# osqp/OSQP.jl

Measured on AMD Instinct MI355X. Metric: ADMM iterations/sec, higher is better.
Workload: dtype f64; 1 GPU; rand-1e6; n=1000000, m=1000000, nnz_A=1000000000, nnz_P_full=1000749500, nnz_P_triu=500874750, backend=pcg, check_termination=25, adaptive_rho_interval=50, instances=1

## Files before the change

include/osqp_amd.h:

```cpp
#ifndef OSQP_AMD_H
#define OSQP_AMD_H

#include <stddef.h>

#ifdef __cplusplus
extern "C" {
#endif

typedef long long c_int;
typedef double    c_float;

#define OSQP_INFTY 1e30

enum osqp_linsys_solver_type {
  QDLDL_SOLVER       = 0,
  MKL_PARDISO_SOLVER = 1,
  AMD_PCG_SOLVER     = 2,
  AMD_DIRECT_SOLVER  = 3
};

#define OSQP_DUAL_INFEASIBLE_INACCURATE    (4)
#define OSQP_PRIMAL_INFEASIBLE_INACCURATE  (3)
#define OSQP_SOLVED_INACCURATE             (2)
#define OSQP_SOLVED                        (1)
// ... 190 lines not shown

c_int osqp_warm_start_x(OSQPWorkspace *work, const c_float *x);
c_int osqp_warm_start_y(OSQPWorkspace *work, const c_float *y);
c_int osqp_warm_start(OSQPWorkspace *work, const c_float *x, const c_float *y);


enum osqp_amd_problem_kind {
  OSQP_AMD_GEN_RANDOM_QP = 0,
  OSQP_AMD_GEN_LASSO     = 1,
  OSQP_AMD_GEN_MPC       = 2
};

c_int osqp_amd_setup_generated(OSQPWorkspace **workp, c_int kind, c_int n, c_int per_row,
                               unsigned long long seed, const OSQPSettings *settings);

#define OSQP_AMD_STATS_COUNT 26
c_int osqp_amd_get_stats(const OSQPWorkspace *work, c_float *out, c_int count);

c_float osqp_amd_time_kernel(OSQPWorkspace *work, c_int which, c_int reps);

typedef struct osqp_amd_comm osqp_amd_comm;
typedef int (*osqp_amd_allgather_fn)(void *ctx, double *host_buf, long long count);
c_int osqp_amd_comm_create_host(osqp_amd_comm **out, c_int rank, c_int world, osqp_amd_allgather_fn fn, void *ctx);
c_int osqp_amd_comm_unique_id(void *out128, const char *librccl_path);
c_int osqp_amd_comm_create_rccl(osqp_amd_comm **out, c_int rank, c_int world, const void *unique_id,
                                const char *librccl_path);
c_int osqp_amd_comm_destroy(osqp_amd_comm *comm);
c_int osqp_amd_comm_all_gather(osqp_amd_comm *comm, c_float *dev_buf, c_int count);
c_int osqp_amd_comm_info(const osqp_amd_comm *comm, c_int *rank, c_int *world, c_int *transport_ranks);
c_int osqp_amd_setup_sharded(OSQPWorkspace **workp, const OSQPData *data, const OSQPSettings *settings,
                             osqp_amd_comm *comm);
// ... 130 lines not shown
```

osqp.jl_amd/csrc/abi.hip:

```cpp
#include "engine.hpp"
#include "symbolic.hpp"

#include <cstring>
#include <thread>
#include <atomic>
#include <cmath>

using namespace oq;

namespace {

struct Impl {
  Engine eng;
  OSQPData data;
  OSQPSettings settings;
  OSQPSolution solution;
  OSQPInfo info;
};

Engine *E(OSQPWorkspace *w) { return &((Impl *)w->impl)->eng; }

struct DeviceGuard {
  int prev = -1;
  explicit DeviceGuard(int want) {
// ... 664 lines not shown
  v[11] = e.lin->trisolve_bytes();
  v[12] = e.A.panel.active ? (e.A.panel.wide ? 3.0 : 2.0) : 0.0;
  v[13] = e.comm ? (c_float)e.comm->world : 1.0;
  v[14] = e.comm ? e.comm->exchanges : 0.0;
  v[15] = e.comm ? e.comm->bytes : 0.0;
  v[16] = (c_float)e.n;
  v[17] = (c_float)e.m;
  v[18] = e.compact ? 1.0 : 0.0;
  v[19] = e.lin->supernode_levels();
  v[20] = (c_float)g_device_peak;
  v[21] = (c_float)e.tree_restarts;
  v[22] = e.lin->multifrontal();
  v[23] = e.lin->lean_setup();
  v[24] = (c_float)dev_va_reserved();
  v[25] = e.lin->dense_block();
  c_int k = 0;
  for (; k < count && k < OSQP_AMD_STATS_COUNT; k++) out[k] = v[k];
  return k;
}

c_float osqp_amd_time_kernel(OSQPWorkspace *w, c_int which, c_int reps) {
  if (!w || reps <= 0) return -1.0;
  OQ_ON_DEVICE(w);
  c_float result = -1.0;
  guarded([&]() {
    Engine &e = *E(w);
    hipStream_t s = e.stream;
    if (which == 3) { result = e.lin->time_solve((int)reps); return 0; }
    if (which == 5) adjoint_moved_on(w, true);
    const double *xin = e.comm ? e.gn.get() : e.x.get(), *yin = e.comm ? e.gm.get() : e.y.get();
    auto run = [&]() {
      switch (which) {
      case 0: spmv(e.A, xin, e.tm2.get(), nullptr, 0.0, 0.0, nullptr, s); break;
      case 1: spmv(e.At, yin, e.tn2.get(), nullptr, 0.0, 0.0, nullptr, s); break;
      case 2: spmv(e.Pf, xin, e.tn2.get(), nullptr, 0.0, 0.0, nullptr, s); break;
      case 7: if (!e.comm) throw Error(1, "not a sharded workspace"); e.full_n(e.tn.get()); break;
      case 5: e.admm_step(); break;
      case 4:
        admm_update(e.n, e.m, e.st.alpha, e.xz.get(), e.rho.get(), e.rho_inv.get(), e.l.get(),
                    e.u.get(), e.tn.get(), e.tm.get(), e.tm2.get(), e.tn2.get(), e.Ax.get(), s);
        break;
      default: throw Error(1, "unknown kernel id");
// ... 149 lines not shown
```

osqp.jl_amd/csrc/engine.hip:

```cpp
#include "engine.hpp"
#include <csignal>
#include <mutex>

#include <algorithm>
#include <cmath>

namespace oq {

thread_local bool g_unsorted_columns = false;
static thread_local std::string g_last_error;
void set_last_error(const std::string &m) { g_last_error = m; }
const char *last_error_cstr() { return g_last_error.c_str(); }

#define RHO_MIN 1e-6
#define RHO_MAX 1e6
#define MIN_SCALING 1e-4
#define MAX_SCALING 1e4

void update_status(OSQPInfo *info, c_int status_val) {
  const char *s = "unsolved";
  info->status_val = status_val;
  switch (status_val) {
  case OSQP_SOLVED: s = "solved"; break;
  case OSQP_SOLVED_INACCURATE: s = "solved inaccurate"; break;
// ... 369 lines not shown
  HIP_CHECK(hipStreamCreateWithFlags(&stream, hipStreamNonBlocking));
  HIP_CHECK(hipHostMalloc((void **)&h_slots, sizeof(double) * (S_COUNT + 8)));
  h_seq = (unsigned long long *)(h_slots + S_COUNT);
  *h_seq = 0;
  {
    void *dp = nullptr;
    static const bool mapped = !(getenv("OSQP_AMD_MAPPED_SLOTS") && atoi(getenv("OSQP_AMD_MAPPED_SLOTS")) == 0);
    if (mapped && hipHostGetDevicePointer(&dp, h_slots, 0) == hipSuccess && dp) {
      h_slots_dev = (double *)dp;
      h_seq_dev = (unsigned long long *)(h_slots_dev + S_COUNT);
    }
  }
  slots.alloc(S_COUNT); slots.zero(stream);
  partials.alloc(16 * kReduceBlocks);
  flag.alloc(4); flag.zero(stream);
}

__global__ __launch_bounds__(kBlock) void k_csr_cols_descend(int64_t nnz, int rows, const int64_t *__restrict__ rp, const int *__restrict__ col,
                                                             int *__restrict__ flag) {
  const int64_t k = (int64_t)blockIdx.x * kBlock + threadIdx.x;
  if (k < 1 || k >= nnz) return;
  if (col[k - 1] < col[k]) return;
  int lo = 0, hi = rows;
  while (hi - lo > 1) { const int mid = (lo + hi) >> 1; if (rp[mid] <= k) lo = mid; else hi = mid; }
  if (rp[lo] != k) *flag = 1;
}

void Engine::setup_device(int n_, int m_, DevBuf<int64_t> &Pp, DevBuf<int> &Pi, DevBuf<double> &Px, DevBuf<int64_t> &Ap,
                          DevBuf<int> &Ai, DevBuf<double> &Ax_in, DevBuf<double> &q_, DevBuf<double> &l_, DevBuf<double> &u_,
                          const OSQPSettings &s) {
// ... 202 lines not shown
}

void Engine::fetch_host_pattern() {
  if (have_host_pattern) return;
  hP.rows = n; hP.cols = n; hP.p.resize((size_t)n + 1); hP.i.resize(nnzPtriu);
  Pp_keep.download(hP.p.data(), (size_t)n + 1, stream);
  Pi_keep.download(hP.i.data(), nnzPtriu, stream);
  hA.rows = m; hA.cols = n; hA.p.resize((size_t)n + 1); hA.i.resize(nnzA);
  At.rowptr.download(hA.p.data(), (size_t)n + 1, stream);
  At.col.download(hA.i.data(), nnzA, stream);
  sync();
  have_host_pattern = true;
}

void Engine::scale_data() {
  c = 1.0;
  vec_set(D.get(), 1.0, n, stream); vec_set(E.get(), 1.0, m, stream);
  double *Dt = tn.get(), *Et = tm.get();
  double *nP = tn2.get(), *nAc = Px_.get(), *nAr = tm2.get();
  csr_row_absmax(Pf, nP, false, stream);
  if (m > 0) {
    csr_row_absmax(At, nAc, false, stream);
    csr_row_absmax(A, nAr, false, stream);
  }
  double c_pend = 1.0;
  for (int it = 0; it < st.scaling; it++) {
    vec_ruiz_factor(Dt, c_pend, nP, m > 0 ? nAc : nullptr, n, stream);
    vec_ruiz_factor(Et, 1.0, nAr, nullptr, m, stream);
    const double *Dg = full_n(Dt);
    csr_scale_rows_cols(Pf, Dt, Dg, 1, 1.0, stream, n0, c_pend, nP);
// ... 75 lines not shown
  const int want = st.linsys_solver;
  if (comm || want == AMD_PCG_SOLVER) return true;
  const double nnzK = (double)nnzPtriu + (double)nnzA + (double)ng + (double)mg;
  return want != AMD_DIRECT_SOLVER && nnzK > 4e7;
}

void Engine::compact_matrices() {
  if (!lin || lin->kind() != 2) return;
  if (!compact_wanted(nnzA + Pf.nnz)) return;
  if (!compact && (!panel_can_compact(Pf) || (m > 0 && !(panel_can_compact(A) && panel_can_compact(At))))) return;
  if (m > 0) { compact_one(0); compact_one(1); }
  compact_one(2);
}

void Engine::unscale_data() {
  csr_scale_rows_cols(Pf, nullptr, nullptr, 0, cinv, stream);
  const double *Dg = full_n(Dinv.get());
  csr_scale_rows_cols(Pf, Dinv.get(), Dg, 1, 1.0, stream, n0);
  vec_scale_by_vec_scalar(q.get(), Dinv.get(), cinv, n, stream);
  if (m > 0) {
    csr_scale_rows_cols(A, Einv.get(), Dg, 0, 1.0, stream);
    csr_scale_rows_cols(At, Dinv.get(), full_m(Einv.get()), 2, 1.0, stream);
    vec_ew_prod(l.get(), l.get(), Einv.get(), m, stream);
    vec_ew_prod(u.get(), u.get(), Einv.get(), m, stream);
  }
}

void Engine::set_rho_vec() {
  st.rho = std::min(std::max(st.rho, RHO_MIN), RHO_MAX);
  rho_vec_update(m, l.get(), u.get(), ctype.get(), rho.get(), rho_inv.get(), st.rho, 0, flag.get(), stream);
// ... 8 lines not shown
  sync();
  if (comm) changed = agree_max(changed ? 1.0 : 0.0) > 0.0;
  if (changed && lin) return lin->update_rho();
  return 0;
}

int Engine::update_rho(double rho_new) {
  if (rho_new <= 0) return 1;
  st.rho = std::min(std::max(rho_new, RHO_MIN), RHO_MAX);
  rho_vec_update(m, l.get(), u.get(), ctype.get(), rho.get(), rho_inv.get(), st.rho, 2, flag.get(), stream);
  settings_changed();
  return lin ? lin->update_rho() : 0;
}

void Engine::cold_start() {
  x.zero(stream); z.zero(stream); y.zero(stream);
}

int Engine::kkt_solve() {
  double cand = -1.0;
  if (have_res) cand = lambda * std::sqrt(sc_pri * sc_dua);
  else if (have_seed) cand = lambda * g_seed;
  return lin->solve(xz.get(), cand);
}

int Engine::admm_step() {
  admm_iters_total++;
  { const int rc = lin->fused_step(); if (rc >= 0) return rc; }
  admm_rhs(n, m, st.sigma, x.get(), q.get(), z.get(), rho_inv.get(), y.get(), xz.get(), stream);
  int rc = kkt_solve();
  admm_update(n, m, st.alpha, xz.get(), rho.get(), rho_inv.get(), l.get(), u.get(), x.get(), z.get(), y.get(), dx.get(),
              dy.get(), stream);
  return rc;
}

int Engine::chunk_k() const {
  const long long k = st.check_termination;
  if (k >= 2) return (int)k;
  if (k != 0) return 0;
  if (!st.adaptive_rho) return 50;
  return st.adaptive_rho_interval > 1 ? (int)std::min<long long>(st.adaptive_rho_interval, 100) : 0;
}
bool Engine::can_chunk(long long iter, long long max_iter) const {
  static const bool enabled = !(getenv("OSQP_AMD_GRAPH") && atoi(getenv("OSQP_AMD_GRAPH")) == 0);
  const long long k = chunk_k();
  if (!enabled || g_debug_sync || lin->kind() != 0 || k < 2 || st.verbose || st.time_limit != 0.0) return false;
  if ((iter - 1) % k != 0 || iter + k - 1 > max_iter) return false;
  if (st.adaptive_rho && (st.adaptive_rho_interval == 0 || st.adaptive_rho_interval % k != 0)) return false;
  return true;
}

void Engine::drop_chunk_graph() {
  if (chunk_exec) { (void)hipGraphExecDestroy(chunk_exec); chunk_exec = nullptr; chunk_len = 0; }
}
void Engine::settings_changed() {
  drop_chunk_graph();
  if (lin) { if (int rc = lin->flush()) deferred_error = rc; lin->invalidate(); }
}

void Engine::run_chunk() {
  const int k = chunk_k();
  if (chunk_exec && chunk_len != k) { (void)hipGraphExecDestroy(chunk_exec); chunk_exec = nullptr; }
  if (!chunk_exec) {
    hipGraph_t graph = nullptr;
    HIP_CHECK(hipStreamBeginCapture(stream, hipStreamCaptureModeThreadLocal));
    struct CaptureGuard {
      Engine &e; bool armed = true;
      ~CaptureGuard() {
        if (!armed) return;
        e.lin->next_follows = false;
        e.lin->invalidate();
        hipGraph_t g = nullptr;
        (void)hipStreamEndCapture(e.stream, &g);
        if (g) (void)hipGraphDestroy(g);
      }
// ... 12 lines not shown
}

void Engine::residual_evaluation() {
  if (int rc = lin->flush()) {
    if (rc == 6) throw TreeFault();
    deferred_error = rc;
  }
  const double *xg = full_n(x.get());
  spmv(A, xg, Ax.get(), nullptr, 0.0, 0.0, nullptr, stream);
  spmv(Pf, xg, Px_.get(), nullptr, 0.0, 0.0, nullptr, stream);
  if (m > 0) spmv(At, full_m(y.get()), Aty.get(), nullptr, 0.0, 0.0, nullptr, stream);
  residual_norms(n, m, x.get(), z.get(), Ax.get(), Px_.get(), Aty.get(), q.get(), Dinv.get(), Einv.get(), slots.get(),
                 partials.get(), stream);
  fetch_slots(0, 16, (1u << S_XPX) | (1u << S_QX));
  if (lin->flush() == 6) throw TreeFault();
}

void Engine::update_info(long long iter, bool compute_objective) {
  OSQPInfo *info = ws->info;
  residual_evaluation();
  memcpy(res, h_slots, sizeof(double) * 16);
  const bool uns = st.scaling && !st.scaled_termination;
  info->iter = iter;
  if (compute_objective) info->obj_val = obj_from_slots();
  info->pri_res = m == 0 ? 0.0 : (uns ? res[S_PRI_UNS] : res[S_PRI]);
  info->dua_res = uns ? cinv * res[S_DUA_UNS] : res[S_DUA];
  sc_pri = m == 0 ? 0.0 : res[S_PRI];
  sc_dua = res[S_DUA];
  double g = std::sqrt(sc_pri * sc_dua);
  have_res = true;
  if (!have_ref) { g_ref = g; it_ref = iter; have_ref = true; }
  else if (iter - it_ref >= 25) {
    if (g > 0.5 * g_ref) lambda = std::max(0.25 * lambda, 1e-6);
    g_ref = g; it_ref = iter;
  }
  info->solve_time = toc();
// ... 308 lines not shown
  if (st.polish && info->status_val == OSQP_SOLVED) polish();
  if (ws->first_run) info->run_time = info->setup_time + info->solve_time + info->polish_time;
  else info->run_time = info->update_time + info->solve_time + info->polish_time;
  ws->first_run = 0;
  clear_update_time = true;
  rho_update_from_solve = false;
  if (st.verbose && rank() == 0)
    printf("status: %s, iterations: %lld, objective: %.6e, run time: %.3es\n", info->status, (long long)info->iter,
           info->obj_val, info->run_time);
  store_solution();
  *ws->settings = st;
  return 0;
}

double Engine::obj_from_slots_fresh() {
  spmv(Pf, full_n(x.get()), Px_.get(), nullptr, 0.0, 0.0, nullptr, stream);
  reduce_dot(x.get(), Px_.get(), n, partials.get(), slots.get() + S_T4, stream);
  reduce_dot(q.get(), x.get(), n, partials.get(), slots.get() + S_T5, stream);
  fetch_slots(S_T4, 2, 3u);
  double obj = 0.5 * h_slots[S_T4] + h_slots[S_T5];
  if (st.scaling) obj *= cinv;
  return obj;
}

int Engine::iterate(long long iters) {
  tic();
  lin->set_guess(x.get());
  for (long long it = 1; it <= iters; it++) {
    if (can_chunk(it, iters)) { run_chunk(); it += chunk_k() - 1; }
    else admm_step();
    if (st.check_termination && (it % st.check_termination == 0)) update_info(it, false);
  }
  update_info(iters, true);
  sync();
  if (deferred_error) { int rc = deferred_error; deferred_error = 0; return rc; }
  return 0;
}

void Engine::polish() {
  tic();
  ws->info->status_polish = polish_run(*this);
  sync();
  ws->info->polish_time = toc();
}

void Engine::begin_update() {
  if (clear_update_time) { clear_update_time = false; ws->info->update_time = 0.0; }
  tic();
}
void Engine::end_update() { sync(); ws->info->update_time += toc(); }

int Engine::update_lin_cost(const double *q_new, bool dev) {
  begin_update();
  load(q.get(), q_new + n0, n, dev);
  sync();
  if (st.scaling) vec_scale_by_vec_scalar(q.get(), D.get(), c, n, stream);
  reset_info(ws->info);
  end_update();
  return 0;
}

// ... 140 lines not shown
      if (A.compact) scatter(Ax_new, Aidx, kA, A.panel.sval.get(), (const uint32_t *)A_k2pos.get(), A.panel.sval.get(), (const uint32_t *)A_k2pos.get());
      else scatter(Ax_new, Aidx, kA, A.val.get(), A_k2pos.get(), nullptr, nullptr);
    }
  }
  }
  if (st.scaling) scale_data();
  refresh_panels();
  settings_changed();
  int e = lin->update_matrices();
  reset_info(ws->info);
  end_update();
  return e;
}

int Engine::warm_start(const double *xw, const double *yw, bool dev) {
  st.warm_start = 1;
  ws->settings->warm_start = 1;
  if (xw) {
    load(x.get(), xw + n0, n, dev); sync();
    if (st.scaling) vec_ew_prod(x.get(), x.get(), Dinv.get(), n, stream);
    if (m > 0) spmv(A, full_n(x.get()), z.get(), nullptr, 0.0, 0.0, nullptr, stream);
  } else {
    x.zero(stream); z.zero(stream);
  }
  if (yw) {
    load(y.get(), yw + m0, m, dev); sync();
    if (st.scaling) vec_scale_by_vec_scalar(y.get(), Einv.get(), c, m, stream);
  } else {
    y.zero(stream);
  }
// ... 103 lines not shown
```

osqp.jl_amd/csrc/engine.hpp:

```cpp
#pragma once
#include <chrono>
#include <memory>

#include "comm.hpp"
#include "kernels.hpp"

namespace oq {

struct Engine;

struct ModelAdjoint;
void model_adjoint_destroy(ModelAdjoint *a);
struct ModelAdjointDeleter { void operator()(ModelAdjoint *a) const { model_adjoint_destroy(a); } };

struct Linsys {
  virtual ~Linsys() {}
  virtual int kind() const = 0;
  virtual int solve(double *xz, double tol_candidate) = 0;
  virtual int update_rho() = 0;
  virtual int update_matrices() = 0;
  virtual void set_guess(const double *x) {}
  virtual int fused_step() { return -1; }
  bool next_follows = false;
  virtual int flush() { return 0; }
  virtual void invalidate() {}
  virtual double nnzL() const { return 0.0; }
  virtual double levels() const { return 0.0; }
  virtual double supernode_levels() const { return 0.0; }
  virtual double multifrontal() const { return 0.0; }
  virtual double dense_block() const { return 0.0; }
  virtual double lean_setup() const { return 0.0; }
  virtual double trisolve_bytes() const { return 0.0; }
  virtual double factorizations() const { return 0.0; }
  virtual double cg_iters() const { return 0.0; }
  virtual float time_solve(int reps) { return -1.f; }
};
// ... 34 lines not shown
  bool compact = false;
  DevBuf<int64_t> Pp_keep;
  DevBuf<int> Pi_keep;
  int64_t nnzA = 0, nnzPtriu = 0;
  HostCsc hP, hA;
  bool have_host_pattern = false;

  DevBuf<double> q, l, u, D, Dinv, E, Einv, rho, rho_inv;
  DevBuf<int> ctype, flag;
  DevBuf<double> x, z, y, xz, dx, dy, Ax, Px_, Aty, tn, tm, tn2, tm2;
  DevBuf<double> slots, partials;
  double *h_slots = nullptr;
  double *h_slots_dev = nullptr;
  unsigned long long *h_seq = nullptr, *h_seq_dev = nullptr, publish_seq = 0;
  double res[16] = {0};
  double c = 1.0, cinv = 1.0;
  std::vector<double> h_l, h_u;
  DevBuf<double> l_raw, u_raw;
  bool h_l_stale = false, h_u_stale = false;
  DevBuf<int64_t> A_to_sorted_dev;
  long long solves_run = 0;
  long long dev_calls[6] = {0, 0, 0, 0, 0, 0};

  std::unique_ptr<Linsys> lin;

  bool solution_current = false;
  std::unique_ptr<ModelAdjoint, ModelAdjointDeleter> adj;

  double sc_pri = 0, sc_dua = 0, lambda0 = 0.015, lambda = 0.015, g_ref = 0;
  long long it_ref = 0;
// ... 156 lines not shown
```

osqp.jl_amd/csrc/kernels.hip:

```cpp
#include "kernels.hpp"
#include "devutil.hpp"
#include <algorithm>

namespace oq {

thread_local const int *g_skip = nullptr;
int g_debug_sync = getenv("OSQP_AMD_DEBUG") ? atoi(getenv("OSQP_AMD_DEBUG")) : 0;

__global__ __launch_bounds__(kBlock) void k_expand_colptr(int cols, const int64_t *__restrict__ colptr, int64_t nnz,
                                                          int *__restrict__ out) {
  int64_t k = (int64_t)blockIdx.x * kBlock + threadIdx.x;
  if (k >= nnz) return;
  int lo = 0, hi = cols;
  while (hi - lo > 1) {
    int mid = (lo + hi) >> 1;
    if (colptr[mid] <= k) lo = mid; else hi = mid;
  }
  out[k] = lo;
}
void expand_colptr(int cols, const int64_t *colptr, int64_t nnz, int *out, hipStream_t s) {
  if (nnz == 0) return;
  OQ_LAUNCH(k_expand_colptr, dim3(blocks_for(nnz)), dim3(kBlock), 0, s, cols, colptr, nnz, out);
}

// ... 401 lines not shown
    const double v0 = va[k], v1 = va[k + G], v2 = va[k + 2 * G], v3 = va[k + 3 * G];
    a0 += v0 * x[c0]; a1 += v1 * x[c1]; a2 += v2 * x[c2]; a3 += v3 * x[c3];
  }
  for (; k < e; k += G) a0 += va[k] * x[ci[k]];
  double acc = (a0 + a1) + (a2 + a3);
#pragma unroll
  for (int o = G >> 1; o > 0; o >>= 1) acc += __shfl_xor(acc, o, 64);
  if (lane == 0) {
    if (rscale) acc *= rscale[row];
    if (beta != 0.0) acc += beta * y[row];
    if (v) acc += gamma * v[row];
    y[row] = acc;
  }
}

void spmv(const DevCsr &M, const double *x, double *y, const double *rscale, double beta, double gamma, const double *v,
          hipStream_t s, const SpmvExtra *extra) {
  if (M.rows == 0) return;
  if (M.panel.active) { spmv_panel(M, x, y, rscale, beta, gamma, v, s, extra); return; }
  if (extra) throw Error(6, "internal: epilogue extras need the panel kernels");
  const int G = M.group;
  dim3 grid(blocks_for((int64_t)M.rows * G)), block(kBlock);
#define OQ_SPMV(GG) \
  OQ_LAUNCH(k_spmv<GG>, grid, block, 0, s, M.rows, M.rowptr.get(), M.col.get(), M.val.get(), x, y, rscale, beta, gamma, v, g_skip)
  switch (G) {
  case 1: OQ_SPMV(1); break;
  case 2: OQ_SPMV(2); break;
  case 4: OQ_SPMV(4); break;
  case 8: OQ_SPMV(8); break;
  case 16: OQ_SPMV(16); break;
  case 32: OQ_SPMV(32); break;
  default: OQ_SPMV(64); break;
  }
// ... 599 lines not shown
```

osqp.jl_amd/csrc/kernels.hpp:

```cpp
#pragma once
#include <functional>
#include "common.hpp"

namespace oq {

extern thread_local const int *g_skip;
struct SkipScope {
  const int *prev;
  explicit SkipScope(const int *flag) : prev(g_skip) { g_skip = flag; }
  ~SkipScope() { g_skip = prev; }
  SkipScope(const SkipScope &) = delete;
  SkipScope &operator=(const SkipScope &) = delete;
};
void fill_slots(double *slots, int count, double value, hipStream_t s);

void expand_colptr(int cols, const int64_t *colptr, int64_t nnz, int *out, hipStream_t s);
void exclusive_scan(const int64_t *counts, int64_t *out, int64_t n, hipStream_t s);
void csr_from_coo(int rows, int cols, int64_t E, const int *erow, const int *ecol, DevCsr &out,
                  DevBuf<int> &src, hipStream_t s);
void gather_values(int64_t nnz, const int *src, const double *in, double *out, int64_t modulo, hipStream_t s);
void invert_map(int64_t nnz, const int *src, int64_t lo, int64_t hi, int *k2pos, hipStream_t s);
void permute_vals(int64_t nnz, const int64_t *to_sorted, const double *in, double *out, hipStream_t s);
void convert_i64_i32(int64_t n, const int64_t *in, int *out, hipStream_t s);
int pick_group(int rows, int64_t nnz);

struct SpmvExtra {
  double *y2 = nullptr;
  const double *s2 = nullptr;
  const double *dotv = nullptr;
  double *dot_partials = nullptr;
  double *absmax_slot = nullptr;
  const double *e2_x1 = nullptr, *e2_x0 = nullptr, *e2_m1 = nullptr, *e2_m0 = nullptr;
  double *e2_partials = nullptr;
};
void spmv(const DevCsr &M, const double *x, double *y, const double *rscale, double beta, double gamma,
          const double *v, hipStream_t s, const SpmvExtra *extra = nullptr);

bool spmv_pair_ok(const DevCsr &Ma, const DevCsr &Mb);
void spmv_pair(const DevCsr &Ma, const DevCsr &Mb, const double *x, double *ya, const SpmvExtra *extra_a, double *yb, double gamma_b,
               const double *vb, hipStream_t s);

bool panel_wanted(const DevCsr &M);
void panel_build(DevCsr &M, hipStream_t s, uint32_t *slot = nullptr, bool will_compact = false,
                 const std::function<void()> &after_cols = std::function<void()>());
void panel_fill(DevCsr &M, bool with_cols, hipStream_t s, uint32_t *slot = nullptr);
void spmv_panel(const DevCsr &M, const double *x, double *y, const double *rscale, double beta, double gamma,
                const double *v, hipStream_t s, const SpmvExtra *extra = nullptr);
bool panel_can_compact(const DevCsr &M);
void panel_compact(DevCsr &M);
// ... 69 lines not shown
```

osqp.jl_amd/csrc/panel.hip:

```cpp
#include <algorithm>
#include <type_traits>

#include "kernels.hpp"
#include <functional>
#include "devutil.hpp"

namespace oq {

namespace {

constexpr int kThreads = 1024;
#ifndef OQ_SELL_BATCH
#define OQ_SELL_BATCH 16
#endif
constexpr int kBatch = OQ_SELL_BATCH;
constexpr int kWaves = kThreads / 64;
constexpr int kTileRowsMax = 3968;
constexpr int kSortN = 4096;
constexpr int64_t kLenMax = 0x7FFFF;

int env_int(const char *name, int dflt) { const char *e = getenv(name); return e ? atoi(e) : dflt; }
int panel_shift() { return env_int("OSQP_AMD_PANEL_SHIFT", 14); }
int panel_tile_nnz() { return env_int("OSQP_AMD_PANEL_TILE_NNZ", 65536); }

// ... 851 lines not shown
  static const bool enabled = !(getenv("OSQP_AMD_SPMV_PAIR") && atoi(getenv("OSQP_AMD_SPMV_PAIR")) == 0);
  return enabled && A.active && B.active && !A.wide && !B.wide && A.shift == B.shift && Ma.cols == Mb.cols && A.ntiles + B.ntiles <= 2048;
}
void spmv_pair(const DevCsr &Ma, const DevCsr &Mb, const double *x, double *ya, const SpmvExtra *extra_a, double *yb, double gamma_b,
               const double *vb, hipStream_t s) {
  auto side = [](const DevCsr &M) {
    const DevPanel &P = M.panel;
    SellSide t;
    t.rows = M.rows; t.cols = M.cols; t.B = P.B; t.Gp = P.Gp; t.ntiles = P.ntiles;
    t.tile_g = P.tile_g.get(); t.tile_r0 = P.tile_r0.get(); t.tile_r1 = P.tile_r1.get(); t.unit_s0 = P.unit_s0.get(); t.unit_ns = P.unit_ns.get();
    t.slice_len = P.slice_len.get(); t.slice_rows = P.slice_rows.get(); t.slice_base = P.slice_base.get(); t.scol = P.scol.get();
    t.sval = P.sval.get(); t.partial = P.partial.get();
    return t;
  };
  const DevPanel &A = Ma.panel, &B = Mb.panel;
  with_sell_nt([&](auto nt) {
    constexpr bool kNT = decltype(nt)::value;
    static size_t allowed[64] = {0};
    allow_dynamic_lds((const void *)k_spmv_sell_pair<kNT>, spmv_lds_bytes(A.shift), allowed);
    OQ_LAUNCH(k_spmv_sell_pair<kNT>, dim3(A.ntiles + B.ntiles), dim3(kThreads), spmv_lds_bytes(A.shift), s, side(Ma), side(Mb), A.shift, x, g_skip);
  });
  ReduceSide ra{Ma.rows, A.NG, reduce_grid(Ma.rows), A.partial.get(), ya, 0.0, nullptr, extra_a ? *extra_a : SpmvExtra()};
  ReduceSide rb{Mb.rows, B.NG, reduce_grid(Mb.rows), B.partial.get(), yb, gamma_b, vb, SpmvExtra()};
  OQ_LAUNCH(k_panel_reduce_pair, dim3(ra.grid + rb.grid), dim3(kBlock), 0, s, ra, rb, g_skip);
}

#define OQ_SELL_VISIT(OP, ...)                                                                                                              \
  do {                                                                                                                                      \
    if (P.wide) OQ_LAUNCH((k_sell_visit<uint32_t, OP>), dim3(P.ntiles), dim3(kThreads), 0, s, M.rows, P.shift, P.B, P.Gp, P.tile_g.get(),    \
                          P.tile_r0.get(), P.tile_r1.get(), P.unit_s0.get(), P.unit_ns.get(), P.slice_base.get(), P.slice_len.get(),        \
// ... 59 lines not shown
```

osqp.jl_amd/csrc/pcg.hip:

```cpp
#include "engine.hpp"
#include "devutil.hpp"

#include <cmath>
#include <map>

namespace oq {

namespace {

constexpr int kRefresh = 25;
constexpr int kMaxSpec = 8;
enum { C_DONE0 = 0, C_DONE1 = 1, C_STALL = 2, C_ERR = 3, C_STEPS = 4, C_ITERS = 5, C_STALL_IT = 6, C_COUNT = 8 };

__global__ void k_pcg_begin(int *ctl, const double *slots, const double *cand_p, double *tol_p) {
  if (ctl[C_STALL]) { ctl[C_DONE0] = 1; return; }
  const double bnorm = slots[S_T5], cand = *cand_p;
  const double hi = 1e-2 * bnorm, lo = 1e-13 * bnorm + 1e-300;
  double tol = hi;
  if (cand >= 0.0) tol = cand;
  if (!(tol < hi)) tol = hi;
  if (tol < lo) tol = lo;
  *tol_p = tol;
  const double rn = slots[S_T1];
  if (rn != rn) { ctl[C_ERR] = 1; ctl[C_STALL] = 1; ctl[C_DONE0] = 1; return; }
// ... 220 lines not shown

__global__ __launch_bounds__(kBlock) void k_extrap_partials(int n, const double *__restrict__ x1, const double *__restrict__ x0,
                                                            const double *__restrict__ Mx1, const double *__restrict__ Mx0,
                                                            const double *__restrict__ b, double *__restrict__ partials,
                                                            const int *__restrict__ skip) {
  if (skip && *skip) return;
  double num = 0.0, den = 0.0;
  for (int i = blockIdx.x * kBlock + threadIdx.x; i < n; i += gridDim.x * kBlock) {
    const double e = x1[i] - x0[i], m1 = Mx1[i];
    num += e * (b[i] - m1);
    den += e * (m1 - Mx0[i]);
  }
  num = block_sum(num);
  den = block_sum(den);
  if (threadIdx.x == 0) { partials[R_DOT + blockIdx.x] = num; partials[R_AUX + blockIdx.x] = den; }
}

struct Pcg : Linsys {
  Engine &e;
  DevBuf<double> xs, r, zz, p, w, t, u, b1, dinv, Axs, Mxs, xs0, Axs0, Mxs0;
  DevBuf<double> qv, sA;
  DevBuf<int> sr_counter;
  bool sr_on = false, sr_first = true;
  bool extrapolate = true, have_prev = false;
  long long total_iters = 0;
  int max_iter = 20000;
  double rel_tol = -1.0;
  bool carried_valid = false;
  int since_refresh = 0;
  bool fused_on = false;
// ... 48 lines not shown
    hipStream_t s = e.stream;
    const double *vg = e.full_n(v);
    const double *tg = nullptr;
    if (e.m > 0) {
      spmv(e.A, vg, Av, nullptr, 0.0, 0.0, nullptr, s);
      vec_ew_prod(t.get(), e.rho.get(), Av, e.m, s);
      tg = e.full_m_begin(t.get());
    }
    spmv(e.Pf, vg, out, nullptr, 0.0, e.st.sigma, v, s);
    if (e.m > 0) {
      e.full_m_end();
      spmv(e.At, tg, out, nullptr, 1.0, 0.0, nullptr, s);
    }
  }

  int solve(double *xz, double cand) override {
    if (int rc = flush()) return rc;
    hipStream_t s = e.stream;
    const int n = e.n, m = e.m;
    double *slots = e.slots.get();
    if (m > 0) {
      vec_ew_prod(t.get(), e.rho.get(), xz + n, m, s);
      spmv(e.At, e.full_m(t.get()), b1.get(), nullptr, 0.0, 1.0, xz, s);
    } else {
      vec_copy(b1.get(), xz, n, s);
    }
    HIP_CHECK(hipMemsetAsync(slots + S_T0, 0, sizeof(double) * 6, s));
    reduce_absmax(b1.get(), nullptr, n, slots + S_T5, s);
    if (!carried_valid || ++since_refresh >= kRefresh) {
      apply_M(xs.get(), Axs.get(), Mxs.get());
      carried_valid = true;
      since_refresh = 0;
    }
    if (extrapolate) {
      if (have_prev) {
        pcg_extrap_dots(n, xs.get(), xs0.get(), Mxs.get(), Mxs0.get(), b1.get(), e.partials.get(), slots + S_T2, slots + S_T3, s);
        e.combine_slots(S_T2, 2, 3u);
        pcg_extrapolate3(xs.get(), xs0.get(), Mxs.get(), Mxs0.get(), n, Axs.get(), Axs0.get(), m, slots + S_T2, slots + S_T3, s);
      } else {
        vec_copy(xs0.get(), xs.get(), n, s); vec_copy(Mxs0.get(), Mxs.get(), n, s);
        if (m > 0) vec_copy(Axs0.get(), Axs.get(), m, s);
        have_prev = true;
      }
    }
    pcg_init_residual(n, b1.get(), Mxs.get(), dinv.get(), r.get(), zz.get(), p.get(), e.partials.get(), slots + S_T0,
// ... 21 lines not shown
                    rz_new + 1, s);
      e.combine_slots(S_T0 + 2 * (1 - cur), 2, 1u);
      pcg_update_p(n, rz_new, rz, zz.get(), p.get(), s);
      e.read_slots(S_T0, 5);
      if (!(e.h_slots[S_T4] > 0.0)) { status = 5; carried_valid = false; break; }
      rn = e.h_slots[S_T1 + 2 * (1 - cur)];
      cur = 1 - cur;
      it++;
    }
    total_iters += it;
    vec_copy2(xz, xs.get(), n, xz + n, Axs.get(), m, s);
    return status;
  }
  int update_rho() override { int rc = flush(); precond(); carried_valid = false; have_prev = false; rhs_ready = false; return rc; }
  int update_matrices() override { int rc = flush(); precond(); carried_valid = false; have_prev = false; rhs_ready = false; return rc; }
  void set_guess(const double *x) override { (void)flush(); vec_copy(xs.get(), x, e.n, e.stream); carried_valid = false; have_prev = false; rhs_ready = false; }

  Publish pub_next;
  DevBuf<int> spec_flag;
  bool spec_now = false;
  double spec_cand = -1.0;
  double need_one = 1.0;
  void start_solve(bool hp, bool refresh, bool async) {
    hipStream_t s = e.stream;
    const int n = e.n, m = e.m;
    double *slots = e.slots.get(), *xz = e.xz.get(), *part = e.partials.get();
    int *flags = async ? ctl.get() : nullptr;
    sr_first = true;
    if (fused_on) {
      if (!(rhs_ready && !async))
        OQ_LAUNCH(k_pcg_rhs, dim3(blocks_for((int64_t)n + m)), dim3(kBlock), 0, s, n, m, e.st.sigma, e.x.get(), e.q.get(), e.z.get(),
                  e.rho.get(), e.rho_inv.get(), e.y.get(), xz, t.get(), slots, g_skip);
      rhs_ready = false;
      SpmvExtra ex;
      ex.absmax_slot = slots + S_T5;
      const bool ext = extrapolate && hp;
      static const bool fuse_e2 = !(getenv("OSQP_AMD_PCG_FUSE_EXTRAP") && atoi(getenv("OSQP_AMD_PCG_FUSE_EXTRAP")) == 0);
      const bool e2 = ext && !refresh && fuse_e2;
      if (e2) { ex.e2_x1 = xs.get(); ex.e2_x0 = xs0.get(); ex.e2_m1 = Mxs.get(); ex.e2_m0 = Mxs0.get(); ex.e2_partials = part + R_DOT; }
      spmv(e.At, t.get(), b1.get(), nullptr, 0.0, 1.0, xz, s, &ex);
      if (refresh) apply_M(xs.get(), Axs.get(), Mxs.get());
      if (ext && !e2) OQ_LAUNCH(k_extrap_partials, dim3(kReduceBlocks), dim3(kBlock), 0, s, n, xs.get(), xs0.get(), Mxs.get(), Mxs0.get(), b1.get(), part, g_skip);
      if (extrapolate)
        OQ_LAUNCH(k_pcg_start, dim3(kReduceBlocks), dim3(kBlock), 0, s, n, m, ext ? 1 : 0, xs.get(), xs0.get(), Mxs.get(), Mxs0.get(), Axs.get(),
                  Axs0.get(), b1.get(), dinv.get(), r.get(), zz.get(), p.get(), part, g_skip);
      else
        pcg_init_residual(n, b1.get(), Mxs.get(), dinv.get(), r.get(), zz.get(), p.get(), part + R_RZ, slots + S_T0, slots + S_T1, s);
      if (extrapolate)
        OQ_LAUNCH(k_pcg_finish_start, dim3(1), dim3(kBlock), 0, s, (const double *)part, slots, flags, (const double *)dctl.get(), dctl.get() + 1,
                  async ? Publish() : pub_next, (!async && spec_now) ? spec_flag.get() : (int *)nullptr, spec_cand, g_skip);
      else if (async)
        OQ_LAUNCH(k_pcg_begin, dim3(1), dim3(1), 0, s, flags, (const double *)slots, (const double *)dctl.get(), dctl.get() + 1);
      return;
    }
    admm_rhs(n, m, e.st.sigma, e.x.get(), e.q.get(), e.z.get(), e.rho_inv.get(), e.y.get(), xz, s);
    if (m > 0) {
      vec_ew_prod(t.get(), e.rho.get(), xz + n, m, s);
      spmv(e.At, t.get(), b1.get(), nullptr, 0.0, 1.0, xz, s);
    } else {
      vec_copy(b1.get(), xz, n, s);
    }
    fill_slots(slots + S_T0, 6, 0.0, s);
    reduce_absmax(b1.get(), nullptr, n, slots + S_T5, s);
    if (refresh) apply_M(xs.get(), Axs.get(), Mxs.get());
    if (extrapolate) {
      if (hp) {
        pcg_extrap_dots(n, xs.get(), xs0.get(), Mxs.get(), Mxs0.get(), b1.get(), part, slots + S_T2, slots + S_T3, s);
        pcg_extrapolate3(xs.get(), xs0.get(), Mxs.get(), Mxs0.get(), n, Axs.get(), Axs0.get(), m, slots + S_T2, slots + S_T3, s);
      } else {
        vec_copy(xs0.get(), xs.get(), n, s); vec_copy(Mxs0.get(), Mxs.get(), n, s);
        if (m > 0) vec_copy(Axs0.get(), Axs.get(), m, s);
      }
    }
    pcg_init_residual(n, b1.get(), Mxs.get(), dinv.get(), r.get(), zz.get(), p.get(), part, slots + S_T0, slots + S_T1, s);
    if (async) {
      SkipScope none(nullptr);
      OQ_LAUNCH(k_pcg_begin, dim3(1), dim3(1), 0, s, flags, (const double *)slots, (const double *)dctl.get(), dctl.get() + 1);
    }
  }
// ... 79 lines not shown
      finish_step();
    }
  }

  int step_sync() {
    double cand = -1.0;
    if (e.have_res) cand = e.lambda * std::sqrt(e.sc_pri * e.sc_dua);
    else if (e.have_seed) cand = e.lambda * e.g_seed;
    const bool refresh = !carried_valid || since_refresh + 1 >= kRefresh;
    const bool self_publish = fused_on && extrapolate;
    pub_next = self_publish ? e.begin_publish() : Publish();
    static const bool spec_allowed = !(getenv("OSQP_AMD_PCG_SPEC") && atoi(getenv("OSQP_AMD_PCG_SPEC")) == 0);
    const bool spec = spec_allowed && self_publish && pub_next.host_slots && max_iter > 0 && need_one >= 0.5;
    if (spec && spec_flag.n == 0) spec_flag.alloc(1);
    spec_now = spec; spec_cand = cand;
    start_solve(have_prev, refresh, false);
    spec_now = false;
    const Publish pub_start = pub_next;
    Publish pub_first;
    if (spec) {
      pub_first = pub_next = e.begin_publish();
      SkipScope on_verdict(spec_flag.get());
      cg_iteration(0, false);
    }
    if (refresh) { carried_valid = true; since_refresh = 0; } else since_refresh++;
    if (extrapolate) have_prev = true;
    if (pub_start.host_slots) e.wait_publish(pub_start); else e.read_slots(S_T0, 6);
    const double bnorm = e.h_slots[S_T5];
    const double hi = 1e-2 * bnorm, lo = 1e-13 * bnorm + 1e-300;
    double tol = hi;
    if (cand >= 0.0) tol = cand;
    if (!(tol < hi)) tol = hi;
// ... 15 lines not shown
      if (pub_it.host_slots) e.wait_publish(pub_it); else e.read_slots(S_T0, 5);
      if (!(e.h_slots[S_T4] > 0.0)) { status = 5; carried_valid = false; break; }
      rn = e.h_slots[S_T1 + 2 * (1 - cur)];
      cur = 1 - cur;
      it++;
    }
    need_one = 0.9 * need_one + (it > 0 ? 0.1 : 0.0);
    total_iters += it;
    static const bool fuse_rhs = !(getenv("OSQP_AMD_PCG_FUSE_RHS") && atoi(getenv("OSQP_AMD_PCG_FUSE_RHS")) == 0);
    finish_step(fuse_rhs && fused_on && status == 0);
    return status;
  }

  int fused_step() override {
    if (!async_on) return fused_on ? step_sync() : -1;
    hipStream_t s = e.stream;
    double cand = -1.0;
    if (e.have_res) cand = e.lambda * std::sqrt(e.sc_pri * e.sc_dua);
    else if (e.have_seed) cand = e.lambda * e.g_seed;
    if (cand != cand_dev) {
      if (issued) { if (int rc = flush()) return rc; }
      HIP_CHECK(hipMemcpyAsync(dctl.get(), &cand, sizeof(double), hipMemcpyHostToDevice, s));
      HIP_CHECK(hipStreamSynchronize(s));
      cand_dev = cand;
    }
    bool refresh = !carried_valid || since_refresh + 1 >= kRefresh;
    issue(spec, have_prev, refresh);
    return 0;
  }
  void issue(int c, bool hp, bool refresh) {
// ... 236 lines not shown
```

Before: 90.13 iterations/s.

## Reuse residual-evaluation A·x and P·x products to seed PCG and objective

After: 89.96 iterations/s. No clear change (-0.2%).

```diff
diff --git a/include/osqp_amd.h b/include/osqp_amd.h
--- a/include/osqp_amd.h
+++ b/include/osqp_amd.h
@@ -228,7 +228,7 @@
 c_int osqp_amd_setup_generated(OSQPWorkspace **workp, c_int kind, c_int n, c_int per_row,
                                unsigned long long seed, const OSQPSettings *settings);
 
-#define OSQP_AMD_STATS_COUNT 26
+#define OSQP_AMD_STATS_COUNT 27
 c_int osqp_amd_get_stats(const OSQPWorkspace *work, c_float *out, c_int count);
 
 c_float osqp_amd_time_kernel(OSQPWorkspace *work, c_int which, c_int reps);
diff --git a/osqp.jl_amd/csrc/abi.hip b/osqp.jl_amd/csrc/abi.hip
--- a/osqp.jl_amd/csrc/abi.hip
+++ b/osqp.jl_amd/csrc/abi.hip
@@ -702,6 +702,7 @@
   v[23] = e.lin->lean_setup();
   v[24] = (c_float)dev_va_reserved();
   v[25] = e.lin->dense_block();
+  v[26] = (c_float)g_spmv_products.load(std::memory_order_relaxed);
   c_int k = 0;
   for (; k < count && k < OSQP_AMD_STATS_COUNT; k++) out[k] = v[k];
   return k;
@@ -714,6 +715,7 @@
   guarded([&]() {
     Engine &e = *E(w);
     hipStream_t s = e.stream;
+    e.moved();
     if (which == 3) { result = e.lin->time_solve((int)reps); return 0; }
     if (which == 5) adjoint_moved_on(w, true);
     const double *xin = e.comm ? e.gn.get() : e.x.get(), *yin = e.comm ? e.gm.get() : e.y.get();
diff --git a/osqp.jl_amd/csrc/engine.hip b/osqp.jl_amd/csrc/engine.hip
--- a/osqp.jl_amd/csrc/engine.hip
+++ b/osqp.jl_amd/csrc/engine.hip
@@ -407,6 +407,8 @@
   slots.alloc(S_COUNT); slots.zero(stream);
   partials.alloc(16 * kReduceBlocks);
   flag.alloc(4); flag.zero(stream);
+  static const bool reuse = !(getenv("OSQP_AMD_PCG_REUSE") && atoi(getenv("OSQP_AMD_PCG_REUSE")) == 0);
+  reuse_products = reuse && !comm;
 }
 
 __global__ __launch_bounds__(kBlock) void k_csr_cols_descend(int64_t nnz, int rows, const int64_t *__restrict__ rp, const int *__restrict__ col,
@@ -639,6 +641,7 @@
 }
 
 void Engine::scale_data() {
+  moved();
   c = 1.0;
   vec_set(D.get(), 1.0, n, stream); vec_set(E.get(), 1.0, m, stream);
   double *Dt = tn.get(), *Et = tm.get();
@@ -744,6 +747,7 @@
 }
 
 void Engine::unscale_data() {
+  moved();
   csr_scale_rows_cols(Pf, nullptr, nullptr, 0, cinv, stream);
   const double *Dg = full_n(Dinv.get());
   csr_scale_rows_cols(Pf, Dinv.get(), Dg, 1, 1.0, stream, n0);
@@ -782,6 +786,7 @@
 }
 
 void Engine::cold_start() {
+  moved();
   x.zero(stream); z.zero(stream); y.zero(stream);
 }
 
@@ -794,6 +799,7 @@
 
 int Engine::admm_step() {
   admm_iters_total++;
+  eval_current = false;
   { const int rc = lin->fused_step(); if (rc >= 0) return rc; }
   admm_rhs(n, m, st.sigma, x.get(), q.get(), z.get(), rho_inv.get(), y.get(), xz.get(), stream);
   int rc = kkt_solve();
@@ -822,11 +828,13 @@
   if (chunk_exec) { (void)hipGraphExecDestroy(chunk_exec); chunk_exec = nullptr; chunk_len = 0; }
 }
 void Engine::settings_changed() {
+  moved();
   drop_chunk_graph();
   if (lin) { if (int rc = lin->flush()) deferred_error = rc; lin->invalidate(); }
 }
 
 void Engine::run_chunk() {
+  moved();
   const int k = chunk_k();
   if (chunk_exec && chunk_len != k) { (void)hipGraphExecDestroy(chunk_exec); chunk_exec = nullptr; }
   if (!chunk_exec) {
@@ -869,12 +877,17 @@
                  partials.get(), stream);
   fetch_slots(0, 16, (1u << S_XPX) | (1u << S_QX));
   if (lin->flush() == 6) throw TreeFault();
+  memcpy(eval_slots, h_slots, sizeof(double) * 16);
+  if (reuse_products) {
+    eval_current = true;
+    if (lin->guess_is_x) lin->guess_products = true;
+  }
 }
 
 void Engine::update_info(long long iter, bool compute_objective) {
   OSQPInfo *info = ws->info;
-  residual_evaluation();
-  memcpy(res, h_slots, sizeof(double) * 16);
+  if (!eval_current) residual_evaluation();
+  memcpy(res, eval_slots, sizeof(double) * 16);
   const bool uns = st.scaling && !st.scaled_termination;
   info->iter = iter;
   if (compute_objective) info->obj_val = obj_from_slots();
@@ -1213,7 +1226,7 @@
 }
 
 double Engine::obj_from_slots_fresh() {
-  spmv(Pf, full_n(x.get()), Px_.get(), nullptr, 0.0, 0.0, nullptr, stream);
+  if (!eval_current) spmv(Pf, full_n(x.get()), Px_.get(), nullptr, 0.0, 0.0, nullptr, stream);
   reduce_dot(x.get(), Px_.get(), n, partials.get(), slots.get() + S_T4, stream);
   reduce_dot(q.get(), x.get(), n, partials.get(), slots.get() + S_T5, stream);
   fetch_slots(S_T4, 2, 3u);
@@ -1238,12 +1251,15 @@
 
 void Engine::polish() {
   tic();
+  moved();
   ws->info->status_polish = polish_run(*this);
+  moved();
   sync();
   ws->info->polish_time = toc();
 }
 
 void Engine::begin_update() {
+  moved();
   if (clear_update_time) { clear_update_time = false; ws->info->update_time = 0.0; }
   tic();
 }
@@ -1414,6 +1430,7 @@
 }
 
 int Engine::warm_start(const double *xw, const double *yw, bool dev) {
+  moved();
   st.warm_start = 1;
   ws->settings->warm_start = 1;
   if (xw) {
diff --git a/osqp.jl_amd/csrc/engine.hpp b/osqp.jl_amd/csrc/engine.hpp
--- a/osqp.jl_amd/csrc/engine.hpp
+++ b/osqp.jl_amd/csrc/engine.hpp
@@ -20,6 +20,7 @@
   virtual int update_rho() = 0;
   virtual int update_matrices() = 0;
   virtual void set_guess(const double *x) {}
+  bool guess_is_x = false, guess_products = false;
   virtual int fused_step() { return -1; }
   bool next_follows = false;
   virtual int flush() { return 0; }
@@ -84,6 +85,13 @@
   double *h_slots_dev = nullptr;
   unsigned long long *h_seq = nullptr, *h_seq_dev = nullptr, publish_seq = 0;
   double res[16] = {0};
+  bool eval_current = false;
+  double eval_slots[16] = {0};
+  bool reuse_products = true;
+  void moved() {
+    eval_current = false;
+    if (lin) lin->guess_is_x = lin->guess_products = false;
+  }
   double c = 1.0, cinv = 1.0;
   std::vector<double> h_l, h_u;
   DevBuf<double> l_raw, u_raw;
diff --git a/osqp.jl_amd/csrc/kernels.hip b/osqp.jl_amd/csrc/kernels.hip
--- a/osqp.jl_amd/csrc/kernels.hip
+++ b/osqp.jl_amd/csrc/kernels.hip
@@ -439,9 +439,12 @@
   }
 }
 
+std::atomic<long long> g_spmv_products{0};
+
 void spmv(const DevCsr &M, const double *x, double *y, const double *rscale, double beta, double gamma, const double *v,
           hipStream_t s, const SpmvExtra *extra) {
   if (M.rows == 0) return;
+  g_spmv_products.fetch_add(1, std::memory_order_relaxed);
   if (M.panel.active) { spmv_panel(M, x, y, rscale, beta, gamma, v, s, extra); return; }
   if (extra) throw Error(6, "internal: epilogue extras need the panel kernels");
   const int G = M.group;
diff --git a/osqp.jl_amd/csrc/kernels.hpp b/osqp.jl_amd/csrc/kernels.hpp
--- a/osqp.jl_amd/csrc/kernels.hpp
+++ b/osqp.jl_amd/csrc/kernels.hpp
@@ -1,4 +1,5 @@
 #pragma once
+#include <atomic>
 #include <functional>
 #include "common.hpp"
 
@@ -33,6 +34,7 @@
   const double *e2_x1 = nullptr, *e2_x0 = nullptr, *e2_m1 = nullptr, *e2_m0 = nullptr;
   double *e2_partials = nullptr;
 };
+extern std::atomic<long long> g_spmv_products;
 void spmv(const DevCsr &M, const double *x, double *y, const double *rscale, double beta, double gamma,
           const double *v, hipStream_t s, const SpmvExtra *extra = nullptr);
 
diff --git a/osqp.jl_amd/csrc/panel.hip b/osqp.jl_amd/csrc/panel.hip
--- a/osqp.jl_amd/csrc/panel.hip
+++ b/osqp.jl_amd/csrc/panel.hip
@@ -889,6 +889,7 @@
     return t;
   };
   const DevPanel &A = Ma.panel, &B = Mb.panel;
+  g_spmv_products.fetch_add(2, std::memory_order_relaxed);
   with_sell_nt([&](auto nt) {
     constexpr bool kNT = decltype(nt)::value;
     static size_t allowed[64] = {0};
diff --git a/osqp.jl_amd/csrc/pcg.hip b/osqp.jl_amd/csrc/pcg.hip
--- a/osqp.jl_amd/csrc/pcg.hip
+++ b/osqp.jl_amd/csrc/pcg.hip
@@ -258,6 +258,16 @@
   num = block_sum(num);
   den = block_sum(den);
   if (threadIdx.x == 0) { partials[R_DOT + blockIdx.x] = num; partials[R_AUX + blockIdx.x] = den; }
+}
+
+__global__ __launch_bounds__(kBlock) void k_pcg_add_scaled(int n, const double *__restrict__ a, double gamma, const double *__restrict__ v,
+                                                           double *__restrict__ out, const int *__restrict__ skip) {
+  if (skip && *skip) return;
+  const int i = blockIdx.x * kBlock + threadIdx.x;
+  if (i >= n) return;
+  double acc = a[i];
+  acc += gamma * v[i];
+  out[i] = acc;
 }
 
 struct Pcg : Linsys {
@@ -336,7 +346,26 @@
     }
   }
 
+  bool start_from_eval = false;
+  bool take_start_products() {
+    const bool have = guess_products;
+    guess_is_x = guess_products = false;
+    return have;
+  }
+  void carry_from_evaluation() {
+    hipStream_t s = e.stream;
+    const int n = e.n, m = e.m;
+    if (m > 0) {
+      vec_copy(Axs.get(), e.Ax.get(), m, s);
+      vec_ew_prod(t.get(), e.rho.get(), Axs.get(), m, s);
+    }
+    OQ_LAUNCH(k_pcg_add_scaled, dim3(blocks_for(n)), dim3(kBlock), 0, s, n, (const double *)e.Px_.get(), e.st.sigma, (const double *)xs.get(),
+              Mxs.get(), g_skip);
+    if (m > 0) spmv(e.At, t.get(), Mxs.get(), nullptr, 1.0, 0.0, nullptr, s);
+  }
+
   int solve(double *xz, double cand) override {
+    const bool from_eval = take_start_products();
     if (int rc = flush()) return rc;
     hipStream_t s = e.stream;
     const int n = e.n, m = e.m;
@@ -350,7 +379,7 @@
     HIP_CHECK(hipMemsetAsync(slots + S_T0, 0, sizeof(double) * 6, s));
     reduce_absmax(b1.get(), nullptr, n, slots + S_T5, s);
     if (!carried_valid || ++since_refresh >= kRefresh) {
-      apply_M(xs.get(), Axs.get(), Mxs.get());
+      if (from_eval) carry_from_evaluation(); else apply_M(xs.get(), Axs.get(), Mxs.get());
       carried_valid = true;
       since_refresh = 0;
     }
@@ -402,7 +431,13 @@
   }
   int update_rho() override { int rc = flush(); precond(); carried_valid = false; have_prev = false; rhs_ready = false; return rc; }
   int update_matrices() override { int rc = flush(); precond(); carried_valid = false; have_prev = false; rhs_ready = false; return rc; }
-  void set_guess(const double *x) override { (void)flush(); vec_copy(xs.get(), x, e.n, e.stream); carried_valid = false; have_prev = false; rhs_ready = false; }
+  void set_guess(const double *x) override {
+    (void)flush();
+    vec_copy(xs.get(), x, e.n, e.stream);
+    carried_valid = false; have_prev = false; rhs_ready = false;
+    guess_is_x = !e.comm && x == e.x.get();
+    guess_products = guess_is_x && e.eval_current;
+  }
 
   Publish pub_next;
   DevBuf<int> spec_flag;
@@ -427,7 +462,7 @@
       const bool e2 = ext && !refresh && fuse_e2;
       if (e2) { ex.e2_x1 = xs.get(); ex.e2_x0 = xs0.get(); ex.e2_m1 = Mxs.get(); ex.e2_m0 = Mxs0.get(); ex.e2_partials = part + R_DOT; }
       spmv(e.At, t.get(), b1.get(), nullptr, 0.0, 1.0, xz, s, &ex);
-      if (refresh) apply_M(xs.get(), Axs.get(), Mxs.get());
+      if (refresh) { if (start_from_eval && !async) carry_from_evaluation(); else apply_M(xs.get(), Axs.get(), Mxs.get()); }
       if (ext && !e2) OQ_LAUNCH(k_extrap_partials, dim3(kReduceBlocks), dim3(kBlock), 0, s, n, xs.get(), xs0.get(), Mxs.get(), Mxs0.get(), b1.get(), part, g_skip);
       if (extrapolate)
         OQ_LAUNCH(k_pcg_start, dim3(kReduceBlocks), dim3(kBlock), 0, s, n, m, ext ? 1 : 0, xs.get(), xs0.get(), Mxs.get(), Mxs0.get(), Axs.get(),
@@ -450,7 +485,7 @@
     }
     fill_slots(slots + S_T0, 6, 0.0, s);
     reduce_absmax(b1.get(), nullptr, n, slots + S_T5, s);
-    if (refresh) apply_M(xs.get(), Axs.get(), Mxs.get());
+    if (refresh) { if (start_from_eval && !async) carry_from_evaluation(); else apply_M(xs.get(), Axs.get(), Mxs.get()); }
     if (extrapolate) {
       if (hp) {
         pcg_extrap_dots(n, xs.get(), xs0.get(), Mxs.get(), Mxs0.get(), b1.get(), part, slots + S_T2, slots + S_T3, s);
@@ -560,8 +595,9 @@
     const bool spec = spec_allowed && self_publish && pub_next.host_slots && max_iter > 0 && need_one >= 0.5;
     if (spec && spec_flag.n == 0) spec_flag.alloc(1);
     spec_now = spec; spec_cand = cand;
+    start_from_eval = take_start_products();
     start_solve(have_prev, refresh, false);
-    spec_now = false;
+    spec_now = false; start_from_eval = false;
     const Publish pub_start = pub_next;
     Publish pub_first;
     if (spec) {
@@ -607,6 +643,7 @@
 
   int fused_step() override {
     if (!async_on) return fused_on ? step_sync() : -1;
+    (void)take_start_products();
     hipStream_t s = e.stream;
     double cand = -1.0;
     if (e.have_res) cand = e.lambda * std::sqrt(e.sc_pri * e.sc_dua);
```
